# sen-ye/dmvae

Measured on AMD Instinct MI355X. Metric: images/sec DMVAE train step @256x256, higher is better.
Workload: dtype bf16

## Files before the change

dmvae_amd/_lib.py:

```python
from __future__ import annotations

import ctypes
import os
from ctypes import POINTER, Structure, c_char_p, c_double, c_float, c_int, c_int32, c_longlong, c_size_t, c_uint, c_ulonglong, c_void_p

_HERE = os.path.dirname(os.path.abspath(__file__))
LIB_PATH = os.environ.get("DMVAE_LIB") or os.path.join(_HERE, "libdmvae_hip.so")


class ConvDesc(Structure):
    _fields_ = [("n", c_int32), ("h", c_int32), ("w", c_int32), ("cin", c_int32), ("cout", c_int32),
                ("ks", c_int32), ("upsample", c_int32), ("act", c_int32), ("out_f32", c_int32), ("stride", c_int32), ("transposed", c_int32),
                ("w_layout", c_int32)]


class PackEntry(Structure):
    _fields_ = [("src", c_void_p), ("dst", c_void_p), ("dst2", c_void_p),
                ("cout", c_int32), ("cin", c_int32), ("T", c_int32), ("rows_pad", c_int32), ("cols_pad", c_int32), ("mode", c_int32), ("subpixel", c_int32),
                ("reserved", c_int32), ("start", c_ulonglong), ("count", c_ulonglong)]


class WtEntry(Structure):
    _fields_ = [("src", c_void_p), ("dst", c_void_p), ("N", c_int32), ("K", c_int32), ("start", c_uint), ("tiles_x", c_uint)]

# ... 34 lines not shown
    "dmvae_gemm_nt_batched": (c_int, [c_void_p] * 5 + [c_int] * 4 + [c_longlong] * 3 + [c_int, c_int, c_void_p]),
    "dmvae_gemm_tn_batched_workspace": (c_size_t, [c_int, c_int, c_int, c_int]),
    "dmvae_gemm_tn_batched": (c_int, [c_void_p] * 4 + [c_size_t] + [c_int] * 4 + [c_longlong] * 3 + [c_float, c_int, c_void_p]),
    "dmvae_set_dynamic": (c_int, [c_int]),
    "dmvae_linear_rows_supported": (c_int, [c_int, c_int, c_int]),
    "dmvae_linear_rows_bf16": (c_int, [c_void_p] * 4 + [c_int] * 10 + [c_void_p]),
    "dmvae_linear_rows_wgrad": (c_int, [c_void_p] * 4 + [c_int] * 6 + [c_void_p]),
    "dmvae_linear_bf16": (c_int, [c_void_p] * 4 + [c_int] * 10 + [c_void_p]),
    "dmvae_linear_bf16_swiglu_pre": (c_int, [c_void_p] * 5 + [c_int] * 9 + [c_void_p]),
    "dmvae_linear_bf16_sk_supported": (c_int, [c_int] * 5),
    "dmvae_linear_bf16_sk_workspace": (c_size_t, [c_int] * 5),
    "dmvae_linear_bf16_sk": (c_int, [c_void_p] * 5 + [c_size_t] + [c_int] * 11 + [c_void_p]),
    "dmvae_linear_bf16_batched_supported": (c_int, [c_int] * 4),
    "dmvae_linear_bf16_batched": (c_int, [c_void_p] * 3 + [c_int] * 7 + [c_longlong] * 3 + [c_int, c_void_p]),
    "dmvae_linear_bf16_plan": (c_int, [c_int, c_int, c_int, POINTER(c_int), POINTER(c_int)]),
    "dmvae_linear_weight_t_kmajor": (c_int, [c_void_p, c_void_p, c_int, c_int, c_void_p]),
    "dmvae_pack_entry_bytes": (c_size_t, []),
    "dmvae_pack_weights_batched": (c_int, [c_void_p, c_int, c_ulonglong, c_int, c_void_p]),
    "dmvae_softmax_rows_fwd": (c_int, [c_void_p, c_void_p, c_int, c_int, c_float, c_void_p]),
    "dmvae_softmax_rows_bwd": (c_int, [c_void_p, c_void_p, c_void_p, c_int, c_int, c_float, c_void_p]),
    "dmvae_transpose_bf16": (c_int, [c_void_p, c_void_p, c_int, c_int, c_int, c_void_p]),
    "dmvae_pack_conv_weight": (c_int, [c_void_p, c_void_p] + [c_int] * 6 + [c_void_p]),
    "dmvae_pack_conv_weight_v2": (c_int, [c_void_p, c_void_p, c_void_p] + [c_int] * 6 + [c_void_p]),
    "dmvae_conv_halo_applies": (c_int, [POINTER(ConvDesc)]),
    "dmvae_conv_kmajor_applies": (c_int, [POINTER(ConvDesc)]),
    "dmvae_subpixel_weight": (c_int, [c_void_p, c_void_p, c_int, c_int, c_void_p]),
    "dmvae_subpixel_weight_fold": (c_int, [c_void_p, c_void_p, c_int, c_int, c_int, c_void_p]),
    "dmvae_colsum_bf16": (c_int, [c_void_p, c_void_p, c_void_p, c_size_t, c_size_t, c_int, c_int, c_void_p]),
    "dmvae_conv_out_wgrad_workspace": (c_size_t, [c_int, c_int, c_int, c_int, c_int]),
    "dmvae_conv_out_wgrad": (c_int, [c_void_p, c_void_p, c_void_p, c_void_p, c_size_t, c_int, c_int, c_int, c_int, c_int, c_int, c_void_p]),
# ... 209 lines not shown
```

dmvae_amd/csrc/common.h:

```cpp
#pragma once
#include <hip/hip_runtime.h>
#include <stdint.h>

typedef __bf16 bf16;
typedef __attribute__((ext_vector_type(8))) __bf16 bf16x8;
typedef __attribute__((ext_vector_type(4))) __bf16 bf16x4;
typedef __attribute__((ext_vector_type(2))) __bf16 bf16x2;
typedef __attribute__((ext_vector_type(4))) short s16x4;
typedef __attribute__((ext_vector_type(16))) float f32x16;
typedef __attribute__((ext_vector_type(4))) float f32x4;
typedef __attribute__((ext_vector_type(2))) float f32x2;

#define GPTR(p) ((const __attribute__((address_space(1))) void*)(p))
#define LPTR(p) ((__attribute__((address_space(3))) void*)(p))

static __device__ uint4 dmvae_zero_page[4];

void dmvae_set_error(const char* fmt, ...);
#define DMVAE_CHECK_ARG(cond, ...) do { if (!(cond)) { dmvae_set_error(__VA_ARGS__); return -22; } } while (0)
#define DMVAE_CHECK_LAUNCH() do { hipError_t e_ = hipGetLastError(); if (e_ != hipSuccess) { dmvae_set_error("%s:%d launch failed: %s", __FILE__, __LINE__, hipGetErrorString(e_)); return -5; } } while (0)

static inline int grid_for(size_t n, int block, int cap) {
  size_t g = (n + block - 1) / block;
  return (int)(g > (size_t)cap ? cap : (g < 1 ? 1 : g));
// ... 26 lines not shown
}
__device__ __forceinline__ s16x4 tr_read_ordered(const char* p) {
  return __builtin_amdgcn_ds_read_tr16_b64_v4i16((__attribute__((address_space(3))) s16x4*)(p));
}

__device__ __forceinline__ float wave_sum(float v) {
#pragma unroll
  for (int o = 32; o > 0; o >>= 1) v += __shfl_xor(v, o, 64);
  return v;
}
__device__ __forceinline__ float bf2f(bf16 v) { return (float)v; }
__device__ __forceinline__ float sigmoidf_(float x) { return __builtin_amdgcn_rcpf(1.0f + __expf(-x)); }
__device__ __forceinline__ float sigmoid_exact(float x) { return 1.0f / (1.0f + expf(-x)); }

__device__ __forceinline__ float dmvae_gelu_f(float x) {
  const float z = fabsf(x) * 0.70710678118654752f;
  const float t = __builtin_amdgcn_rcpf(__builtin_fmaf(0.3275911f, z, 1.0f));
  float p = __builtin_fmaf(1.061405429f, t, -1.453152027f);
  p = __builtin_fmaf(p, t, 1.421413741f);
  p = __builtin_fmaf(p, t, -0.284496736f);
  p = __builtin_fmaf(p, t, 0.254829592f);
  const float e = p * t * __expf(-z * z);
  return 0.5f * x * (x < 0.f ? e : 2.0f - e);
}

__device__ __forceinline__ unsigned xcd_remap(unsigned flat, unsigned total) {
  const unsigned q = total >> 3, r = total & 7u, x = flat & 7u;
  const unsigned start = x < r ? x * (q + 1) : r * (q + 1) + (x - r) * q;
  return start + (flat >> 3);
}

__device__ __forceinline__ bf16x8 dmvae_ldnt8(const bf16* p) {
  return __builtin_nontemporal_load(reinterpret_cast<const bf16x8*>(p));
}
__device__ __forceinline__ unsigned dmvae_pack_bf16x2(float a, float b) {
  bf16x2 t = {(bf16)a, (bf16)b};
  return *reinterpret_cast<unsigned*>(&t);
}
// ... 28 lines not shown
```

dmvae_amd/csrc/gemm_pp.hip:

```cpp
#include "common.h"
#include "dmvae_hip.h"
#include <cstdlib>
#include <type_traits>

constexpr int GEMM_MAXBUF = 6;

namespace dmvae_gemm_pp {

struct Args {
  const bf16* x;
  const bf16* w;
  const void* bias;
  void* y;
  int M, N, K, lda, ldw, ldy;
  int act, bias_bf16;
  int H;
  unsigned wbytes;
  unsigned wsRow, wsK;
  int ntn, total;
  float inv_ntn;
  int tpb;
  float inv_tpb;
  unsigned sA, sB, sY, xbytes, ybytes;
  unsigned long long* dbg;
  int V, skS, T;
  float* slabs;
  unsigned* counters;
  unsigned slab_bytes;
  void* y2;
  int ldy2;
};

constexpr int SK_COHERENT = 1 | 16;

template <int TM, int TP, int WM, int WP, bool OUT_F32, int NBUF, bool BATCHED = false, bool SK = false>
__global__ __launch_bounds__(WM * WP * 64) void gemm_pp_kernel(Args a) {
#if __HIP_DEVICE_COMPILE__
  constexpr int PF = NBUF - 1;
  static_assert(!(SK && BATCHED) && !(SK && OUT_F32), "SK: single product, bf16 result");
  constexpr int CL = TM / WM / 16, BT = TP / WP / 16;
  constexpr int NW = WM * WP;
  static_assert(NW == 8 && CL * 16 * WM == TM && BT * 16 * WP == TP && CL * BT <= 32 && (CL == 4 || CL == 6 || CL == 8), "wave grid");
  constexpr int TILE_A = TM * 64, TILE_B = TP * 64, SLOT = TILE_A + TILE_B, RING = NBUF * SLOT;
  constexpr int NPA = (TM / 16 + NW - 1) / NW, NPB = (TP / 16 + NW - 1) / NW, NP = NPA + NPB;
  constexpr int CW = CL * 16;
  constexpr int BIAS_OFF = RING, DUMP_OFF = RING + 2048;
// ... 29 lines not shown
    if constexpr (BATCHED) {
      int b = (int)((float)wid * a.inv_tpb);
      int r = wid - b * a.tpb;
      if (r < 0) { b--; r += a.tpb; }
      if (r >= a.tpb) { b++; r -= a.tpb; }
      b0 = __builtin_amdgcn_readfirstlane(b);
      wid = r;
      offA = (unsigned)b0 * a.sA; offB = (unsigned)b0 * a.sB;
    }
    int mt = (int)((float)wid * inv_ntn);
    int nt = wid - mt * a.ntn;
    if (nt < 0) { mt--; nt += a.ntn; }
    if (nt >= a.ntn) { mt++; nt -= a.ntn; }
    m0 = __builtin_amdgcn_readfirstlane(mt) * TP;
    n0 = __builtin_amdgcn_readfirstlane(nt) * TM;
#pragma unroll
    for (int p = 0; p < NPA; p++) {
      const int rl = (wave * NPA + p) * 16 + (lane_c >> 2);
      const int wmr = rl / CW, r = rl % CW, i = r >> 4, c = r & 15;
      int n = n0 + wmr * CW + CL * c + i;
      bool n_ok = n < a.N;
      if (gated) {
        const int hid = (n0 >> 1) + wmr * (CW / 2) + (CL / 2) * c + (i % (CL / 2));
        n = (i < CL / 2 ? 0 : a.H) + hid;
        n_ok = hid < a.H;
      }
      const int ch = (lane_c & 3) ^ swz64(rl);
      vA[p] = (live && rl < TM && n_ok) ? (unsigned)n * a.wsRow + ch * 16u + offA : SENT;
    }
#pragma unroll
// ... 108 lines not shown
    __builtin_amdgcn_sched_barrier(0);
#pragma unroll
    for (int i = 0; i < CL; i++)
#pragma unroll
      for (int j = 0; j < BT; j++)
        asm volatile("v_mfma_f32_16x16x32_bf16 %0, %1, %2, %0" : "+a"(acc[i][j]) : "v"(tf[j]), "v"(wf[i]));
    __builtin_amdgcn_sched_barrier(0);
    __builtin_amdgcn_s_barrier();
    __builtin_amdgcn_sched_barrier(0);
  };
  using W_NO = std::integral_constant<int, -1>; using W_0 = std::integral_constant<int, 0>;
  using W_ST = std::integral_constant<int, (PF - 1) * NP>; using W_TL = std::integral_constant<int, (PF - 1) * NP + 1>;
  using M0_ = std::integral_constant<int, 0>;
  static_assert((PF - 1) * NP + 1 < 64, "vmcnt is a 6-bit counter");

  unsigned work = blockIdx.x;
  if constexpr (SK) { uc = next_unit(); work = (unsigned)uc.tile; }
  {
    unsigned vBiasC;
    calc(work, vAc, vBc, vBiasC, m0c, n0c, b0c);
    issue_bias(vBiasC, 0);
  }
#pragma unroll
  for (int u = 0; u < PF; u++) issue_k(vAc, vBc, (unsigned)(u + (SK ? uc.kb : 0)), u * SLOT);
  wait_vmcnt<0>();

  int tix = 0;
  auto stamp = [&](int k) { if (a.dbg && tid == 0 && tix < 4) a.dbg[((size_t)blockIdx.x * 4 + tix) * 8 + k] = __builtin_amdgcn_s_memtime(); };
  while (work < (unsigned)a.total) {
    stamp(0);
    __builtin_amdgcn_s_barrier();
    {
      const char* bl = smem + BIAS_OFF + par * 1024;
      int lane_b = lane;
      asm volatile("" : "+v"(lane_b));
      const int col = gated ? wm * (CW / 2) + (CL / 2) * (lane_b & 15) : wm * CW + CL * (lane_b & 15);
      const int hop = gated ? TM / 2 - CL / 2 : 0;
      float bv[8] = {0.f, 0.f, 0.f, 0.f, 0.f, 0.f, 0.f, 0.f};
      if (!a.bias || (SK && uc.p != 0)) {
      } else if (a.bias_bf16) {
#pragma unroll
        for (int h = 0; h < CL / 2; h++) {
          const bf16x2 b2 = *reinterpret_cast<const bf16x2*>(bl + (col + (h >= CL / 4 ? hop : 0)) * 2 + h * 4);
// ... 146 lines not shown
                  } else {
                    const unsigned p1 = dmvae_pack_bf16x2(v[0], v[1]), p2 = dmvae_pack_bf16x2(v[2], v[3]);
                    __builtin_amdgcn_raw_buffer_store_b32(p1, rY2, ok2 ? e1 : SENT, 0, 0);
                    __builtin_amdgcn_raw_buffer_store_b32(p2, rY2, ok2 ? e2 : SENT, 0, 0);
                    asm volatile("s_nop 0" :: "v"(p1), "v"(p2));
                  }
                }
              }
#pragma unroll
              for (int i = 0; i < CL / 2; i++) {
                const float x1 = (float)(bf16)v[i], x2 = (float)(bf16)v[CL / 2 + i];
                v[i] = (float)(bf16)(x1 * sigmoidf_(x1)) * x2;
              }
            } else if constexpr (ACT != 0) {
#pragma unroll
              for (int i = 0; i < CL; i++) {
                const float x = (float)(bf16)v[i];
                v[i] = ACT == 5 ? dmvae_gelu_f(x) : x * sigmoidf_(x);
              }
            }
            const int m = row0 + j * 16 + r;
            const bool ok = c_ok && m < a.M;
            const unsigned eo = (unsigned)m * (unsigned)a.ldy + (unsigned)col;
            if constexpr (ACT == 6) {
              if constexpr (CL == 8 && !OUT_F32) {
                const u32x2 o = {dmvae_pack_bf16x2(v[0], v[1]), dmvae_pack_bf16x2(v[2], v[3])};
                __builtin_amdgcn_raw_buffer_store_b64(o, rY, ok ? eo * 2u : SENT, ysoff, 0);
                asm volatile("s_nop 0" :: "v"(o));
              } else if constexpr (CL == 4 && !OUT_F32) {
                const unsigned o = dmvae_pack_bf16x2(v[0], v[1]);
                __builtin_amdgcn_raw_buffer_store_b32(o, rY, ok ? eo * 2u : SENT, ysoff, 0);
                asm volatile("s_nop 0" :: "v"(o));
              }
            } else if constexpr (OUT_F32 && CL == 6) {
// ... 58 lines not shown
#pragma unroll
    for (int p = 0; p < NPA; p++) vAc[p] = vAn[p];
#pragma unroll
    for (int p = 0; p < NPB; p++) vBc[p] = vBn[p];
    m0c = m0n; n0c = n0n; b0c = b0n;
    if constexpr (SK) uc = un;
    par ^= 1;
  }
#endif
}

template <int TM, int TP, int WM, int WP, bool F32, bool BATCHED = false>
int launch(Args a, hipStream_t st, int batch = 1) {
  a.ntn = (a.N + TM - 1) / TM;
  a.tpb = ((a.M + TP - 1) / TP) * a.ntn;
  a.total = a.tpb * batch;
  DMVAE_CHECK_ARG(a.total > 0 && a.total < (1 << 24) && (long long)a.tpb * batch < (1 << 24),
                  "linear_bf16: %lld output tiles (the kernel's tile index arithmetic is exact below 2^24)", (long long)a.tpb * batch);
  a.inv_ntn = 1.0f / (float)a.ntn;
  a.inv_tpb = 1.0f / (float)a.tpb;
  const unsigned grid = a.total > 256 ? 256u : (unsigned)a.total;
  constexpr int slot = (TM + TP) * 64;
  constexpr int fit = (160 * 1024 - 3 * 1024) / slot;
  constexpr int nbuf = fit > GEMM_MAXBUF ? GEMM_MAXBUF : fit;
  static_assert(nbuf >= 4, "LDS");
  constexpr int lds = nbuf * slot + 3 * 1024;
  DMVAE_LDS_OPTIN(lds, gemm_pp_kernel<TM, TP, WM, WP, F32, nbuf, BATCHED>);
  hipLaunchKernelGGL((gemm_pp_kernel<TM, TP, WM, WP, F32, nbuf, BATCHED>), dim3(grid), dim3(WM * WP * 64), lds, st, a);
  DMVAE_CHECK_LAUNCH();
  return 0;
// ... 31 lines not shown
  const int nK = K >> 5;
  if (tiles > SK_MAX_TILES || tiles * nK >= (1ll << 30)) return false;
  if (splits == 0) return tiles * nK / SK_GRID >= 2 * t.minseg && nK >= 2 * t.minseg;
  return nK / splits >= t.minseg && tiles * splits <= 4096;
}

struct Cfg { int tm, tp; float cost; };
static const Cfg g_cfg[] = {
    {256, 256, 1.00f}, {256, 224, 0.94f}, {256, 192, 0.885f}, {256, 160, 0.80f}, {256, 128, 0.67f},
    {128, 448, 1.02f}, {128, 384, 0.93f}, {128, 256, 0.70f},  {192, 256, 0.90f}, {192, 320, 1.12f},
    {192, 128, 0.54f}, {128, 192, 0.54f},
};
constexpr int NCFG = sizeof(g_cfg) / sizeof(g_cfg[0]);

static int g_forced = -1;
static int plan(int M, int N, int K, bool gated = false) {
  const int forced = g_forced;
  if (forced >= 0 && forced < NCFG && !(gated && g_cfg[forced].tm == 192)) return forced;
  (void)K;
  constexpr int NPLAN = 10;
  int best = 0;
  float best_t = 1e30f;
  for (int c = 0; c < NPLAN; c++) {
    if (gated && g_cfg[c].tm == 192) continue;
    const long long tiles = (long long)((M + g_cfg[c].tp - 1) / g_cfg[c].tp) * ((N + g_cfg[c].tm - 1) / g_cfg[c].tm);
    const float frac = (float)tiles / 256.0f, whole = 0.85f * (float)((tiles + 255) / 256);
    const float t = (frac > whole ? frac : whole) * g_cfg[c].cost;
    if (t < best_t * 0.999f) { best_t = t; best = c; }
  }
  return best;
}

template <bool F32>
static int dispatch(int cfg, const Args& a, hipStream_t st) {
  switch (cfg) {
    case 0: return launch<256, 256, 2, 4, F32>(a, st);
    case 1: return launch<256, 224, 4, 2, F32>(a, st);
    case 2: return launch<256, 192, 2, 4, F32>(a, st);
    case 3: return launch<256, 160, 4, 2, F32>(a, st);
    case 4: return launch<256, 128, 4, 2, F32>(a, st);
    case 5: return launch<128, 448, 2, 4, F32>(a, st);
    case 6: return launch<128, 384, 2, 4, F32>(a, st);
    case 7: return launch<128, 256, 2, 4, F32>(a, st);
// ... 3 lines not shown
    default: return launch<128, 192, 2, 4, F32>(a, st);
  }
}

}

static unsigned long long* g_gemm_dbg = nullptr;
extern "C" void dmvae_debug_gemm_timing(void* buf) { g_gemm_dbg = (unsigned long long*)buf; }
extern "C" void dmvae_debug_gemm_cfg(int cfg) { dmvae_gemm_pp::g_forced = cfg; }

extern "C" int dmvae_linear_bf16_plan(int M, int N, int K, int* tile_cols, int* tile_rows) {
  using namespace dmvae_gemm_pp;
  const int c = plan(M, N, K);
  if (tile_cols) *tile_cols = g_cfg[c].tm;
  if (tile_rows) *tile_rows = g_cfg[c].tp;
  return c;
}

extern "C" int dmvae_linear_bf16_batched_supported(int batch, int M, int N, int K) {
  return (batch > 0 && M >= 64 && N > 0 && N % 8 == 0 && K >= 384 && K % 32 == 0) ? 1 : 0;
}
extern "C" int dmvae_linear_bf16_batched(const void* x, const void* w, void* y, int batch, int M, int N, int K, int lda, int ldw, int ldy, long long sx, long long sw,
                                         long long sy, int out_f32, hipStream_t stream) {
  using namespace dmvae_gemm_pp;
  DMVAE_CHECK_ARG(x && w && y, "linear_bf16_batched: null operand");
  DMVAE_CHECK_ARG(dmvae_linear_bf16_batched_supported(batch, M, N, K), "linear_bf16_batched: need K %% 32 == 0, K >= 384, N %% 8 == 0, M >= 64 (batch %d, M %d, N %d, K %d)",
                  batch, M, N, K);
  DMVAE_CHECK_ARG(lda >= K && ldw >= K && ldy >= N && lda % 8 == 0 && ldw % 8 == 0 && ldy % 8 == 0, "linear_bf16_batched: leading dimensions must cover the rows and be multiples of 8");
  DMVAE_CHECK_ARG(sx >= (long long)M * lda && sw >= (long long)N * ldw && sy >= (long long)M * ldy && sx % 8 == 0 && sw % 8 == 0 && sy % 8 == 0,
                  "linear_bf16_batched: batch strides must cover one product's operand and be multiples of 8 elements");
  const long long xb = ((long long)(batch - 1) * sx + (long long)M * lda) * 2, wb = ((long long)(batch - 1) * sw + (long long)N * ldw) * 2;
  const long long yb = ((long long)(batch - 1) * sy + (long long)M * ldy) * (out_f32 ? 4 : 2);
  DMVAE_CHECK_ARG(xb < (1ll << 31) && wb < (1ll << 31) && yb < (1ll << 31), "linear_bf16_batched: operands are addressed through 32-bit buffer offsets (2 GiB each over the whole batch)");
  Args a;
  a.x = (const bf16*)x; a.w = (const bf16*)w; a.bias = nullptr; a.y = y;
  a.M = M; a.N = N; a.K = K; a.lda = lda; a.ldw = ldw; a.ldy = ldy;
  a.act = 0; a.bias_bf16 = 0; a.H = N / 2; a.ntn = 0; a.total = 0; a.inv_ntn = 0.f; a.dbg = nullptr;
  a.V = a.skS = a.T = 0; a.slabs = nullptr; a.counters = nullptr; a.slab_bytes = 0u; a.y2 = nullptr; a.ldy2 = 0;
  a.wbytes = (unsigned)wb; a.xbytes = (unsigned)xb; a.ybytes = (unsigned)yb;
  a.wsRow = (unsigned)ldw * 2u; a.wsK = 64u;
  a.sA = (unsigned)(sw * 2); a.sB = (unsigned)(sx * 2); a.sY = (unsigned)(sy * (out_f32 ? 4 : 2));
  static const int cand[3] = {0, 4, 7};
  int best = 0;
  float best_t = 1e30f;
  for (int i = 0; i < 3; i++) {
    const Cfg& c = g_cfg[cand[i]];
    const long long tiles = (long long)batch * ((M + c.tp - 1) / c.tp) * ((N + c.tm - 1) / c.tm);
    const float frac = (float)tiles / 256.0f, whole = 0.85f * (float)((tiles + 255) / 256);
    const float t = (frac > whole ? frac : whole) * c.cost;
    if (t < best_t * 0.999f) { best_t = t; best = cand[i]; }
  }
  if (out_f32) {
    if (best == 0) return launch<256, 256, 2, 4, true, true>(a, stream, batch);
// ... 25 lines not shown
  DMVAE_CHECK_ARG(act == 0 || act == 1 || act == 5 || act == 6, "linear_bf16_sk: act must be 0 (none), 1 (SiLU), 5 (GELU) or 6 (SwiGLU over the [x1 | x2] halves of N)");
  DMVAE_CHECK_ARG(act != 6 || N % 16 == 0, "linear_bf16_sk: the SwiGLU epilogue needs N %% 16 == 0");
  const long long wb = w_layout == 1 ? (long long)N * K * 2 : (long long)N * ldw * 2;
  DMVAE_CHECK_ARG((long long)M * lda * 2 < (1ll << 31) && wb < (1ll << 31) && (long long)M * ldy * 2 < (1ll << 31),
                  "linear_bf16_sk: operands are addressed through 32-bit buffer offsets (2 GiB each)");
  const size_t need = dmvae_linear_bf16_sk_workspace(M, N, K, splits, tile);
  DMVAE_CHECK_ARG(workspace_bytes >= need && need - SK_COUNTER_BYTES < (1ull << 32), "linear_bf16_sk: workspace too small (need %zu bytes, see dmvae_linear_bf16_sk_workspace)", need);
  Args a;
  a.x = (const bf16*)x; a.w = (const bf16*)w; a.bias = bias; a.y = y;
  a.M = M; a.N = N; a.K = K; a.lda = lda; a.ldw = ldw; a.ldy = ldy;
  a.act = act; a.bias_bf16 = bias_bf16; a.H = N / 2; a.ntn = 0; a.total = 0; a.inv_ntn = 0.f; a.dbg = g_gemm_dbg;
  a.wbytes = (unsigned)wb; a.tpb = 0; a.inv_tpb = 0.f; a.sA = a.sB = a.sY = a.xbytes = a.ybytes = 0u;
  a.wsRow = w_layout == 1 ? 64u : (unsigned)ldw * 2u;
  a.wsK = w_layout == 1 ? (unsigned)N * 64u : 64u;
  a.y2 = nullptr; a.ldy2 = 0;
  a.counters = (unsigned*)workspace;
  a.slabs = (float*)((char*)workspace + SK_COUNTER_BYTES);
  a.slab_bytes = (unsigned)(need - SK_COUNTER_BYTES);
  return launch_sk(a, splits, tile, stream);
}

static int linear_bf16_impl(const void* x, const void* w, const void* bias, void* y, void* y2, int ldy2, int M, int N, int K, int lda, int ldw, int ldy,
                            int act, int bias_bf16, int out_f32, int w_layout, hipStream_t stream);
extern "C" int dmvae_linear_bf16(const void* x, const void* w, const void* bias, void* y, int M, int N, int K, int lda, int ldw, int ldy,
                                 int act, int bias_bf16, int out_f32, int w_layout, hipStream_t stream) {
  return linear_bf16_impl(x, w, bias, y, nullptr, 0, M, N, K, lda, ldw, ldy, act, bias_bf16, out_f32, w_layout, stream);
}
extern "C" int dmvae_linear_bf16_swiglu_pre(const void* x, const void* w, const void* bias, void* g, void* x12, int M, int N, int K, int lda, int ldw, int ldg,
                                            int ldx12, int bias_bf16, int w_layout, hipStream_t stream) {
  DMVAE_CHECK_ARG(x12 && ldx12 >= N && ldx12 % 8 == 0, "linear_bf16_swiglu_pre: x12 must be given with ldx12 >= N, a multiple of 8");
  return linear_bf16_impl(x, w, bias, g, x12, ldx12, M, N, K, lda, ldw, ldg, 6, bias_bf16, 0, w_layout, stream);
}
static int linear_bf16_impl(const void* x, const void* w, const void* bias, void* y, void* y2, int ldy2, int M, int N, int K, int lda, int ldw, int ldy,
                            int act, int bias_bf16, int out_f32, int w_layout, hipStream_t stream) {
  using namespace dmvae_gemm_pp;
  DMVAE_CHECK_ARG(x && w && y, "linear_bf16: null operand");
  DMVAE_CHECK_ARG(M > 0 && N > 0 && K >= 384 && K % 32 == 0 && N % 8 == 0, "linear_bf16: need K %% 32 == 0, K >= 384 and N %% 8 == 0 (M %d, N %d, K %d)", M, N, K);
  DMVAE_CHECK_ARG(w_layout == 0 || w_layout == 1, "linear_bf16: w_layout must be 0 (row-major [N][ldw]) or 1 (K-tile-major [K / 32][N][32])");
  DMVAE_CHECK_ARG(lda >= K && (w_layout == 1 || ldw >= K) && ldy >= (act == 6 ? N / 2 : N) && lda % 8 == 0 && ldw % 8 == 0 && ldy % 8 == 0,
                  "linear_bf16: leading dimensions must cover the rows and be multiples of 8");
  DMVAE_CHECK_ARG(act == 0 || act == 1 || act == 5 || act == 6, "linear_bf16: act must be 0 (none), 1 (SiLU), 5 (GELU) or 6 (SwiGLU over the [x1 | x2] halves of N)");
  DMVAE_CHECK_ARG(act != 6 || (!out_f32 && N % 16 == 0), "linear_bf16: the SwiGLU epilogue writes bf16 and needs N %% 16 == 0");
  const long long wb = w_layout == 1 ? (long long)N * K * 2 : (long long)N * ldw * 2;
  DMVAE_CHECK_ARG((long long)M * lda * 2 < (1ll << 31) && wb < (1ll << 31) && (long long)M * ldy * (out_f32 ? 4 : 2) < (1ll << 31),
                  "linear_bf16: operands are addressed through 32-bit buffer offsets (2 GiB each)");
  Args a;
  a.x = (const bf16*)x; a.w = (const bf16*)w; a.bias = bias; a.y = y;
  a.M = M; a.N = N; a.K = K; a.lda = lda; a.ldw = ldw; a.ldy = ldy;
  a.act = act; a.bias_bf16 = bias_bf16; a.H = N / 2; a.ntn = 0; a.total = 0; a.inv_ntn = 0.f; a.dbg = g_gemm_dbg;
  a.V = a.skS = a.T = 0; a.slabs = nullptr; a.counters = nullptr; a.slab_bytes = 0u; a.y2 = y2; a.ldy2 = ldy2;
  DMVAE_CHECK_ARG(!y2 || (long long)M * ldy2 * 2 < (1ll << 31), "linear_bf16_swiglu_pre: x12 is addressed through 32-bit buffer offsets (2 GiB)");
  a.wbytes = (unsigned)wb; a.tpb = 0; a.inv_tpb = 0.f; a.sA = a.sB = a.sY = a.xbytes = a.ybytes = 0u;
  a.wsRow = w_layout == 1 ? 64u : (unsigned)ldw * 2u;
  a.wsK = w_layout == 1 ? (unsigned)N * 64u : 64u;
  const int cfg = plan(M, N, K, act == 6);
  return out_f32 ? dispatch<true>(cfg, a, stream) : dispatch<false>(cfg, a, stream);
}
```

dmvae_amd/functional.py:

```python
from __future__ import annotations

from typing import Optional
import os

import weakref

import torch

from . import ops, parity
from .ops import bf16, f32

_EPOCH = [0]


def bump_weight_epoch() -> None:
    _EPOCH[0] += 1


def _epoch_of(w) -> int:
    return getattr(w, "_dmvae_epoch", _EPOCH)[0]


def packed(w: torch.Tensor, for_dgrad: bool = False, rows_pad: int = 0, cols_pad: int = 0, frozen: bool = False,
           transposed: bool = False, subpixel: bool = False, kmajor: bool = False) -> torch.Tensor:
# ... 776 lines not shown
SPLITK = 3
SPLITK_MIN_K = 3072
_SPLITK_ACTIVE = [0]


def _use_splitk(m: int, n: int, k: int) -> int:
    s_ = _SPLITK_ACTIVE[0]
    if s_ < 2 or parity.on() or not (2048 <= m <= 6144) or k < SPLITK_MIN_K:
        return 0
    tiles = ((m + 255) // 256) * ((n + 255) // 256)
    if tiles > 100:
        return 0
    return s_ if ops.linear_sk_supported(m, n, k, s_) else 0


def linear(x: torch.Tensor, w: torch.Tensor, b: Optional[torch.Tensor] = None, act: int = ops.ACT_NONE) -> torch.Tensor:
    bb = None if b is None else (b if b.dtype == bf16 else _bf(b))
    k = x.shape[-1]
    n = w.shape[0]
    m = x.numel() // k
    x = _c(x)
    if x.dtype != bf16:
        x = x.to(bf16)
    if m <= 64 and act in (ops.ACT_NONE, ops.ACT_SILU) and ops.linear_rows_supported(m, n, k) and not parity.on():
        return ops.linear_rows(x.view(m, k), (w if w.dtype == bf16 else _bf(w)).view(n, k), bb, act).view(*x.shape[:-1], n)
    sk = _use_splitk(m, n, k) if act == ops.ACT_NONE else 0
    if sk:
        return ops.linear_sk(x.view(m, k), (w if w.dtype == bf16 else _bf(w)).view(n, k), bb, splits=sk).view(*x.shape[:-1], n)
    if ops.linear_supported(m, n, k) and (act != ops.ACT_SWIGLU or n % 16 == 0):
        if isinstance(w, torch.nn.Parameter) and not w.requires_grad and not hasattr(w, "_dmvae_epoch") and w.dim() == 2:
            return ops.linear_bf16(x, _bf_km(w), bb, act)
        return ops.linear_bf16(x, (w if w.dtype == bf16 else _bf(w)).view(n, k), bb, act)
    wb = w if w.dtype == bf16 else _bf(w)
    x2, w2 = x.view(m, k), wb.view(n, k)
    if k % 32 != 0 or n % 4 != 0:
        kp, np_ = (-k) % 32, (-n) % 4
        x2 = torch.nn.functional.pad(x2, (0, kp))
        w2 = torch.nn.functional.pad(w2, (0, kp, 0, np_))
        bb = None if bb is None else torch.nn.functional.pad(bb, (0, np_))
    y = ops.gemm_nt(x2, w2, None if bb is None else bb.float())[:, :n]
    if act == ops.ACT_GELU:
        y = ops.gelu(y)
    elif act == ops.ACT_SILU:
        y = ops.silu(y)
    elif act == ops.ACT_SWIGLU:
        y = ops.swiglu(_c(y))
    return y.reshape(*x.shape[:-1], y.shape[-1])
# ... 718 lines not shown
```

dmvae_amd/models/vit_fast.py:

```python
import torch
import torch.nn.functional as F

from .. import ops


def patch_embed_gemm(vit, x: torch.Tensor) -> torch.Tensor:
    w = vit.patch_embed.proj.weight
    b_, c, hh, ww = x.shape
    p = w.shape[-1]
    assert hh % p == 0 and ww % p == 0, "image size must be a multiple of the patch size"
    patches = x.view(b_, c, hh // p, p, ww // p, p).permute(0, 2, 4, 1, 3, 5).reshape(b_, (hh // p) * (ww // p), c * p * p)
    if not torch.is_grad_enabled():
        from ..functional import linear
        return linear(patches.to(torch.bfloat16), _w(w).view(w.shape[0], -1), _w(vit.patch_embed.proj.bias))
    from ..functional import LinearFn
    return LinearFn.apply(patches, w.view(w.shape[0], -1), vit.patch_embed.proj.bias)


def _w(p: torch.Tensor) -> torch.Tensor:
    if p.dtype == torch.bfloat16:
        return p
    from ..functional import _bf
    return _bf(p)


@torch.no_grad()
def frozen_forward_features(vit, x: torch.Tensor, key_depths=None, pos_embed=None):
    from ..functional import linear
    t = patch_embed_gemm(vit, x).float()
    t = torch.cat([vit.cls_token.expand(t.shape[0], -1, -1).float(), t], dim=1) + (vit.pos_embed if pos_embed is None else pos_embed).float()
    taps, last_tap = [], (max(key_depths) if key_depths is not None else -1)
    t = t.contiguous()
    b, s, c = t.shape
    hn = ops.layernorm_bf16(t, vit.blocks[0].norm1.weight, vit.blocks[0].norm1.bias, vit.blocks[0].norm1.eps)
    nblk = len(vit.blocks)
    for i, blk in enumerate(vit.blocks):
        nh = blk.attn.num_heads
        hd = c // nh
        qkv = linear(hn, blk.attn.qkv.weight, blk.attn.qkv.bias)
        if hd == 64:
            o = ops.attention_qkv(qkv, nh, hd ** -0.5)
        else:
            from .._stock import require_opt_in
            require_opt_in("vit_fast.forward_features (attention)", f"head dim {hd}: the fused attention kernels take head dim 64")
            qkv = qkv.reshape(b, s, 3, nh, hd).permute(2, 0, 3, 1, 4)
            att = ops.softmax_rows_bf16(qkv[0] @ qkv[1].transpose(-2, -1), hd ** -0.5)
            o = (att @ qkv[2]).transpose(1, 2).reshape(b, s, c)
        o = linear(o, blk.attn.proj.weight, blk.attn.proj.bias)
        hn = ops.scale_residual_layernorm_(t, o.contiguous(), blk.ls1.gamma, blk.norm2.weight, blk.norm2.bias, blk.norm2.eps)
        h = linear(hn, blk.mlp.fc1.weight, blk.mlp.fc1.bias, act=ops.ACT_GELU)
        o = linear(h, blk.mlp.fc2.weight, blk.mlp.fc2.bias)
        if i == last_tap:
            taps.append(ops.scale_residual_(t, o.contiguous(), blk.ls2.gamma))
            return taps
        nxt = vit.blocks[i + 1].norm1 if i + 1 < nblk else vit.norm
        hn = ops.scale_residual_layernorm_(t, o, blk.ls2.gamma, nxt.weight, nxt.bias, nxt.eps)
        if key_depths is not None and i in key_depths:
            taps.append(t.clone())
    if key_depths is not None:
        raise ValueError(f"key_depths {tuple(key_depths)}: the model has {nblk} blocks")
    return hn


def hip_path_supported(vit, seq_len: int) -> bool:
    c = vit.embed_dim
    nh = vit.blocks[0].attn.num_heads
    return c in (256, 384, 512, 768, 1024, 1280, 1536) and c // nh == 64


NOGRAD_FUSED = True


def frozen_taps_with_input_grad(vit, x: torch.Tensor, key_depths, pos_embed=None):
    from ..functional import VitBlockDxFn
    t = patch_embed_gemm(vit, x)
    t = torch.cat([vit.cls_token.expand(t.shape[0], -1, -1).float(), t.float()], dim=1) + (vit.pos_embed if pos_embed is None else pos_embed).float()
    t = t.contiguous()
    taps = []
    for i, blk in enumerate(vit.blocks[:max(key_depths) + 1]):
        t = VitBlockDxFn.apply(t, blk.norm1.weight, blk.norm1.bias, blk.attn.qkv.weight, blk.attn.qkv.bias, blk.attn.proj.weight, blk.attn.proj.bias,
                               blk.ls1.gamma, blk.norm2.weight, blk.norm2.bias, blk.mlp.fc1.weight, blk.mlp.fc1.bias, blk.mlp.fc2.weight,
                               blk.mlp.fc2.bias, blk.ls2.gamma, blk.attn.num_heads, blk.norm1.eps)
        if i in key_depths:
            taps.append(t)
# ... 61 lines not shown
```

dmvae_amd/ops.py:

```python
from __future__ import annotations

import ctypes
import os
from typing import Optional, Sequence, Tuple

import torch

from . import _lib, parity
from ._lib import ConvDesc, check

bf16 = torch.bfloat16
f32 = torch.float32

ACT_NONE, ACT_SILU, ACT_RELU, ACT_RELU_GATE, ACT_LEAKY, ACT_GELU = 0, 1, 2, 3, 4, 5
ACT_SWIGLU = 6


def _stream() -> int:
    return torch.cuda.current_stream().cuda_stream


def _req(t: torch.Tensor, dtype, name: str) -> torch.Tensor:
    if not t.is_cuda:
        raise _lib.DmvaeHipError(f"{name}: expected a GPU tensor; dmvae_amd has no CPU path")
# ... 295 lines not shown
    m = x.numel() // k
    bias_bf16 = 0
    if bias is not None:
        if bias.dtype == bf16:
            bias_bf16 = 1
        _req(bias, bf16 if bias_bf16 else f32, "bias")
        assert bias.numel() == n
    ny = n // 2 if act == ACT_SWIGLU else n
    y = torch.empty(*x.shape[:-1], ny, dtype=f32 if out_f32 else bf16, device=x.device)
    timing = KERNEL_TIMING
    if timing is not None:
        e0 = torch.cuda.Event(enable_timing=True)
        e0.record()
    check(_lib.lib().dmvae_linear_bf16(x.data_ptr(), w.data_ptr(), _ptr(bias), y.data_ptr(), m, n, k, k, k, ny, act, bias_bf16, int(out_f32), int(kmajor),
                                       _stream()), "linear_bf16")
    if timing is not None:
        e1 = torch.cuda.Event(enable_timing=True)
        e1.record()
        timing.append(("gemm_pp_kernel", e0, e1, 2.0 * m * n * k))
    return y


def linear_swiglu_pre(x: torch.Tensor, w: torch.Tensor, bias: Optional[torch.Tensor] = None):
    x = _req(x, bf16, "x")
    w = _req(w, bf16, "w")
    k = x.shape[-1]
    kmajor = w.dim() == 3
    n = w.shape[1] if kmajor else w.shape[0]
    assert (w.shape[0] * 32 == k and w.shape[2] == 32) if kmajor else (w.shape[1] == k), (x.shape, w.shape)
    m = x.numel() // k
# ... 2005 lines not shown
```

include/dmvae_hip.h:

```cpp
#ifndef DMVAE_HIP_H
#define DMVAE_HIP_H

#include <stddef.h>
#include <stdint.h>

#ifdef __cplusplus
extern "C" {
#endif

typedef struct ihipStream_t* dmvae_stream_t;

const char* dmvae_last_error(void);
int dmvae_abi_version(void);


typedef struct dmvae_conv_desc {
  int32_t n, h, w;
  int32_t cin, cout;
  int32_t ks;
  int32_t upsample;
  int32_t act;
  int32_t out_f32;
  int32_t stride;
  int32_t transposed;
// ... 74 lines not shown
size_t dmvae_gemm_tn_batched_workspace(int M, int N, int K, int batch);
int dmvae_gemm_tn_batched(const void* A, const void* B, void* C, void* workspace, size_t workspace_bytes, int M,
                          int N, int K, int batch, long long a_bs, long long b_bs, long long c_bs, float alpha,
                          int out_f32, dmvae_stream_t stream);

int dmvae_linear_rows_supported(int M, int N, int K);
int dmvae_linear_rows_bf16(const void* x, const void* w, const void* bias, void* y, int M, int N, int K, int ldx, int ldw, int ldy, int act,
                           int bias_bf16, int out_f32, int w_layout, dmvae_stream_t stream);
int dmvae_linear_rows_wgrad(const void* dy, const void* x, void* dw, void* db, int M, int N, int K, int lddy, int ldx, int accumulate, dmvae_stream_t stream);

int dmvae_set_dynamic(int on);

int dmvae_linear_bf16(const void* x, const void* w, const void* bias, void* y, int M, int N, int K, int lda, int ldw, int ldy,
                      int act, int bias_bf16, int out_f32, int w_layout, dmvae_stream_t stream);
int dmvae_linear_bf16_plan(int M, int N, int K, int* tile_cols, int* tile_rows);
int dmvae_linear_bf16_batched_supported(int batch, int M, int N, int K);
int dmvae_linear_bf16_batched(const void* x, const void* w, void* y, int batch, int M, int N, int K, int lda, int ldw, int ldy, long long sx, long long sw,
                              long long sy, int out_f32, dmvae_stream_t stream);
int dmvae_linear_bf16_swiglu_pre(const void* x, const void* w, const void* bias, void* g, void* x12, int M, int N, int K, int lda, int ldw, int ldg,
                                 int ldx12, int bias_bf16, int w_layout, dmvae_stream_t stream);

int dmvae_linear_bf16_sk_supported(int M, int N, int K, int splits, int tile);
size_t dmvae_linear_bf16_sk_workspace(int M, int N, int K, int splits, int tile);
int dmvae_linear_bf16_sk(const void* x, const void* w, const void* bias, void* y, void* workspace, size_t workspace_bytes, int splits, int tile,
                         int M, int N, int K, int lda, int ldw, int ldy, int act, int bias_bf16, int w_layout, dmvae_stream_t stream);
int dmvae_linear_weight_t_kmajor(const void* w, void* out, int N, int K, dmvae_stream_t stream);

int dmvae_softmax_rows_fwd(const void* s, void* p, int rows, int cols, float scale, dmvae_stream_t stream);
int dmvae_softmax_rows_bwd(const void* dp, const void* p, void* ds, int rows, int cols, float scale,
                           dmvae_stream_t stream);
// ... 365 lines not shown
```

Before: 502.2.

## Add segmented GEMM mode so ViT fc1 tiles skip CLS rows via strip pass

Adds a segmented linear mode for the frozen ViT feature extractor's fc1 GEMM. Each sequence of s rows has its leading CLS row handled by a small MFMA strip pass run before the main tiled loop. The main tiles then cover only the remaining 256-multiple token rows, so per-image sequences of 257 tokens no longer spill into a partially filled tile. The planner weighs the strip cost against tile savings, and the GELU epilogue is also rewritten with contraction off and an explicit fma.

```diff
diff --git a/dmvae_amd/_lib.py b/dmvae_amd/_lib.py
--- a/dmvae_amd/_lib.py
+++ b/dmvae_amd/_lib.py
@@ -72,6 +72,8 @@
     "dmvae_linear_bf16_batched_supported": (c_int, [c_int] * 4),
     "dmvae_linear_bf16_batched": (c_int, [c_void_p] * 3 + [c_int] * 7 + [c_longlong] * 3 + [c_int, c_void_p]),
     "dmvae_linear_bf16_plan": (c_int, [c_int, c_int, c_int, POINTER(c_int), POINTER(c_int)]),
+    "dmvae_linear_bf16_seg": (c_int, [c_void_p] * 4 + [c_int] * 13 + [c_void_p]),
+    "dmvae_linear_bf16_seg_plan": (c_int, [c_int] * 6 + [POINTER(c_int)] * 3),
     "dmvae_linear_weight_t_kmajor": (c_int, [c_void_p, c_void_p, c_int, c_int, c_void_p]),
     "dmvae_pack_entry_bytes": (c_size_t, []),
     "dmvae_pack_weights_batched": (c_int, [c_void_p, c_int, c_ulonglong, c_int, c_void_p]),
diff --git a/dmvae_amd/csrc/common.h b/dmvae_amd/csrc/common.h
--- a/dmvae_amd/csrc/common.h
+++ b/dmvae_amd/csrc/common.h
@@ -64,14 +64,15 @@
 __device__ __forceinline__ float sigmoid_exact(float x) { return 1.0f / (1.0f + expf(-x)); }
 
 __device__ __forceinline__ float dmvae_gelu_f(float x) {
+#pragma clang fp contract(off)
   const float z = fabsf(x) * 0.70710678118654752f;
   const float t = __builtin_amdgcn_rcpf(__builtin_fmaf(0.3275911f, z, 1.0f));
   float p = __builtin_fmaf(1.061405429f, t, -1.453152027f);
   p = __builtin_fmaf(p, t, 1.421413741f);
   p = __builtin_fmaf(p, t, -0.284496736f);
   p = __builtin_fmaf(p, t, 0.254829592f);
-  const float e = p * t * __expf(-z * z);
-  return 0.5f * x * (x < 0.f ? e : 2.0f - e);
+  const float pt = p * t, ex = __expf(-z * z);
+  return 0.5f * x * (x < 0.f ? pt * ex : __builtin_fmaf(-ex, pt, 2.0f));
 }
 
 __device__ __forceinline__ unsigned xcd_remap(unsigned flat, unsigned total) {
diff --git a/dmvae_amd/csrc/gemm_pp.hip b/dmvae_amd/csrc/gemm_pp.hip
--- a/dmvae_amd/csrc/gemm_pp.hip
+++ b/dmvae_amd/csrc/gemm_pp.hip
@@ -29,7 +29,18 @@
   unsigned slab_bytes;
   void* y2;
   int ldy2;
+  int seg_rows, seg_skip, nseg, seg_tps;
+  float inv_tps;
 };
+
+template <int ACT>
+__device__ __forceinline__ float act_value(float v) {
+  if constexpr (ACT == 0) return v;
+  else {
+    const float x = (float)(bf16)v;
+    return ACT == 5 ? dmvae_gelu_f(x) : x * sigmoidf_(x);
+  }
+}
 
 constexpr int SK_COHERENT = 1 | 16;
 
@@ -89,6 +100,16 @@
     if (nt >= a.ntn) { mt++; nt -= a.ntn; }
     m0 = __builtin_amdgcn_readfirstlane(mt) * TP;
     n0 = __builtin_amdgcn_readfirstlane(nt) * TM;
+    if constexpr (!BATCHED && !SK) {
+      if (a.seg_rows) {
+        const int mtu = __builtin_amdgcn_readfirstlane(mt);
+        int sg = (int)((float)mtu * a.inv_tps);
+        int r = mtu - sg * a.seg_tps;
+        if (r < 0) { sg--; r += a.seg_tps; }
+        if (r >= a.seg_tps) { sg++; r -= a.seg_tps; }
+        m0 = __builtin_amdgcn_readfirstlane(sg * a.seg_rows + a.seg_skip + r * TP);
+      }
+    }
 #pragma unroll
     for (int p = 0; p < NPA; p++) {
       const int rl = (wave * NPA + p) * 16 + (lane_c >> 2);
@@ -227,6 +248,8 @@
   using M0_ = std::integral_constant<int, 0>;
   static_assert((PF - 1) * NP + 1 < 64, "vmcnt is a 6-bit counter");
 
+  int tix = 0;
+  auto stamp = [&](int k) { if (a.dbg && tid == 0 && tix < 4) a.dbg[((size_t)blockIdx.x * 4 + tix) * 8 + k] = __builtin_amdgcn_s_memtime(); };
   unsigned work = blockIdx.x;
   if constexpr (SK) { uc = next_unit(); work = (unsigned)uc.tile; }
   {
@@ -236,10 +259,80 @@
   }
 #pragma unroll
   for (int u = 0; u < PF; u++) issue_k(vAc, vBc, (unsigned)(u + (SK ? uc.kb : 0)), u * SLOT);
+
+  if constexpr (!BATCHED && !SK) {
+    if (a.seg_rows) {
+      stamp(4);
+      constexpr int SD = 12;
+      const int R = a.nseg * a.seg_skip, RB = (R + 15) >> 4, CB = (a.N + 15) >> 4;
+      const int ncl = (CB - (int)blockIdx.x + (int)gridDim.x - 1) / (int)gridDim.x;
+      const int c16 = lane & 15, g4 = lane >> 4;
+      auto strip_row = [&](int s_) -> int { const int sg = s_ / a.seg_skip; return sg * a.seg_rows + (s_ - sg * a.seg_skip); };
+      for (int lu = wave; lu < ncl * RB; lu += NW) {
+        const int ci = lu / RB, rb = lu - ci * RB;
+        const int n = ((int)blockIdx.x + ci * (int)gridDim.x) * 16 + c16;
+        const int s_in = rb * 16 + c16;
+        const unsigned vX = s_in < R ? (unsigned)strip_row(s_in) * (unsigned)a.lda * 2u + (unsigned)g4 * 16u : SENT;
+        const unsigned vW = n < a.N ? (unsigned)n * a.wsRow + (unsigned)g4 * 16u : SENT;
+        float bv = 0.f;
+        if (a.bias) {
+          if (a.bias_bf16) {
+            const unsigned short raw = (unsigned short)__builtin_amdgcn_raw_buffer_load_b16(rBias, n < a.N ? (unsigned)n * 2u : SENT, 0, 0);
+            bv = (float)*reinterpret_cast<const bf16*>(&raw);
+          } else {
+            bv = __builtin_bit_cast(float, __builtin_amdgcn_raw_buffer_load_b32(rBias, n < a.N ? (unsigned)n * 4u : SENT, 0, 0));
+          }
+        }
+        f32x4 sacc = {bv, bv, bv, bv};
+        int k0 = 0;
+        auto steps = [&](auto NBc) __attribute__((always_inline)) {
+          constexpr int NB = decltype(NBc)::value;
+          u32x4 xa[NB], wb[NB];
+#pragma unroll
+          for (int u = 0; u < NB; u++) {
+            xa[u] = __builtin_amdgcn_raw_buffer_load_b128(rB, vX, (unsigned)(k0 + u) * 64u, 0);
+            wb[u] = __builtin_amdgcn_raw_buffer_load_b128(rA, vW, (unsigned)(k0 + u) * a.wsK, 0);
+          }
+          __builtin_amdgcn_sched_barrier(0);
+#pragma unroll
+          for (int u = 0; u < NB; u++)
+            sacc = __builtin_amdgcn_mfma_f32_16x16x32_bf16(*reinterpret_cast<const bf16x8*>(&xa[u]), *reinterpret_cast<const bf16x8*>(&wb[u]), sacc, 0, 0, 0);
+          k0 += NB;
+        };
+#pragma unroll 1
+        while (k0 + SD <= nK) steps(std::integral_constant<int, SD>{});
+        if (k0 + 8 <= nK) steps(std::integral_constant<int, 8>{});
+        if (k0 + 4 <= nK) steps(std::integral_constant<int, 4>{});
+        if (k0 + 2 <= nK) steps(std::integral_constant<int, 2>{});
+        if (k0 < nK) steps(std::integral_constant<int, 1>{});
+        auto put = [&](auto ACTc) __attribute__((always_inline)) {
+          constexpr int ACT = decltype(ACTc)::value;
+#pragma unroll
+          for (int r = 0; r < 4; r++) {
+            const int s_out = rb * 16 + 4 * g4 + r;
+            const bool ok = s_out < R && n < a.N;
+            const unsigned eo = (unsigned)strip_row(s_out) * (unsigned)a.ldy + (unsigned)n;
+            const float v = act_value<ACT>(sacc[r]);
+            if constexpr (OUT_F32) {
+              const unsigned o = __builtin_bit_cast(unsigned, v);
+              __builtin_amdgcn_raw_buffer_store_b32(o, rY, ok ? eo * 4u : SENT, 0, 0);
+              asm volatile("s_nop 0" :: "v"(o));
+            } else {
+              const unsigned short o = (unsigned short)(dmvae_pack_bf16x2(v, 0.f) & 0xffffu);
+              __builtin_amdgcn_raw_buffer_store_b16(o, rY, ok ? eo * 2u : SENT, 0, 0);
+              asm volatile("s_nop 0" :: "v"(o));
+            }
+          }
+        };
+        if (a.act == 0) put(std::integral_constant<int, 0>{});
+        else if (a.act == 5) put(std::integral_constant<int, 5>{});
+        else put(std::integral_constant<int, 1>{});
+      }
+      stamp(5);
+    }
+  }
   wait_vmcnt<0>();
 
-  int tix = 0;
-  auto stamp = [&](int k) { if (a.dbg && tid == 0 && tix < 4) a.dbg[((size_t)blockIdx.x * 4 + tix) * 8 + k] = __builtin_amdgcn_s_memtime(); };
   while (work < (unsigned)a.total) {
     stamp(0);
     __builtin_amdgcn_s_barrier();
@@ -416,10 +509,7 @@
               }
             } else if constexpr (ACT != 0) {
 #pragma unroll
-              for (int i = 0; i < CL; i++) {
-                const float x = (float)(bf16)v[i];
-                v[i] = ACT == 5 ? dmvae_gelu_f(x) : x * sigmoidf_(x);
-              }
+              for (int i = 0; i < CL; i++) v[i] = act_value<ACT>(v[i]);
             }
             const int m = row0 + j * 16 + r;
             const bool ok = c_ok && m < a.M;
@@ -508,6 +598,11 @@
 int launch(Args a, hipStream_t st, int batch = 1) {
   a.ntn = (a.N + TM - 1) / TM;
   a.tpb = ((a.M + TP - 1) / TP) * a.ntn;
+  if (a.seg_rows) {
+    a.seg_tps = (a.seg_rows - a.seg_skip) / TP;
+    a.inv_tps = 1.0f / (float)a.seg_tps;
+    a.tpb = a.nseg * a.seg_tps * a.ntn;
+  }
   a.total = a.tpb * batch;
   DMVAE_CHECK_ARG(a.total > 0 && a.total < (1 << 24) && (long long)a.tpb * batch < (1 << 24),
                   "linear_bf16: %lld output tiles (the kernel's tile index arithmetic is exact below 2^24)", (long long)a.tpb * batch);
@@ -569,9 +664,19 @@
 constexpr int NCFG = sizeof(g_cfg) / sizeof(g_cfg[0]);
 
 static int g_forced = -1;
-static int plan(int M, int N, int K, bool gated = false) {
+struct Seg { int rows, skip, n; };
+constexpr float STRIP_COST = 0.22f;
+static bool seg_fits(const Seg* seg, int M, int tp) {
+  return seg && seg->rows > 0 && seg->skip > 0 && seg->skip < seg->rows && seg->n > 0 && (long long)seg->n * seg->rows == M && (seg->rows - seg->skip) % tp == 0;
+}
+static int plan(int M, int N, int K, bool gated = false, const Seg* seg = nullptr, bool* use_seg = nullptr) {
+  if (use_seg) *use_seg = false;
+  if (gated) seg = nullptr;
   const int forced = g_forced;
-  if (forced >= 0 && forced < NCFG && !(gated && g_cfg[forced].tm == 192)) return forced;
+  if (forced >= 0 && forced < NCFG && !(gated && g_cfg[forced].tm == 192)) {
+    if (use_seg) *use_seg = seg_fits(seg, M, g_cfg[forced].tp);
+    return forced;
+  }
   (void)K;
   constexpr int NPLAN = 10;
   int best = 0;
@@ -581,7 +686,15 @@
     const long long tiles = (long long)((M + g_cfg[c].tp - 1) / g_cfg[c].tp) * ((N + g_cfg[c].tm - 1) / g_cfg[c].tm);
     const float frac = (float)tiles / 256.0f, whole = 0.85f * (float)((tiles + 255) / 256);
     const float t = (frac > whole ? frac : whole) * g_cfg[c].cost;
-    if (t < best_t * 0.999f) { best_t = t; best = c; }
+    if (t < best_t * 0.999f) { best_t = t; best = c; if (use_seg) *use_seg = false; }
+    if (seg_fits(seg, M, g_cfg[c].tp)) {
+      const long long stiles = (long long)seg->n * ((seg->rows - seg->skip) / g_cfg[c].tp) * ((N + g_cfg[c].tm - 1) / g_cfg[c].tm);
+      const long long grid = stiles > 256 ? 256 : stiles;
+      const long long blocks = (((N + 15) / 16 + grid - 1) / grid) * (((long long)seg->n * seg->skip + 15) / 16);
+      const float sfrac = (float)stiles / 256.0f, swhole = 0.85f * (float)((stiles + 255) / 256);
+      const float ts = (sfrac > swhole ? sfrac : swhole) * g_cfg[c].cost + STRIP_COST * (float)((blocks + 7) / 8);
+      if (ts < best_t * 0.999f) { best_t = ts; best = c; if (use_seg) *use_seg = true; }
+    }
   }
   return best;
 }
@@ -615,6 +728,16 @@
   const int c = plan(M, N, K);
   if (tile_cols) *tile_cols = g_cfg[c].tm;
   if (tile_rows) *tile_rows = g_cfg[c].tp;
+  return c;
+}
+extern "C" int dmvae_linear_bf16_seg_plan(int M, int N, int K, int seg_rows, int seg_skip, int nseg, int* tile_cols, int* tile_rows, int* segmented) {
+  using namespace dmvae_gemm_pp;
+  const Seg seg = {seg_rows, seg_skip, nseg};
+  bool us = false;
+  const int c = plan(M, N, K, false, &seg, &us);
+  if (tile_cols) *tile_cols = g_cfg[c].tm;
+  if (tile_rows) *tile_rows = g_cfg[c].tp;
+  if (segmented) *segmented = us ? 1 : 0;
   return c;
 }
 
@@ -638,6 +761,7 @@
   a.M = M; a.N = N; a.K = K; a.lda = lda; a.ldw = ldw; a.ldy = ldy;
   a.act = 0; a.bias_bf16 = 0; a.H = N / 2; a.ntn = 0; a.total = 0; a.inv_ntn = 0.f; a.dbg = nullptr;
   a.V = a.skS = a.T = 0; a.slabs = nullptr; a.counters = nullptr; a.slab_bytes = 0u; a.y2 = nullptr; a.ldy2 = 0;
+  a.seg_rows = a.seg_skip = a.nseg = a.seg_tps = 0; a.inv_tps = 0.f;
   a.wbytes = (unsigned)wb; a.xbytes = (unsigned)xb; a.ybytes = (unsigned)yb;
   a.wsRow = (unsigned)ldw * 2u; a.wsK = 64u;
   a.sA = (unsigned)(sw * 2); a.sB = (unsigned)(sx * 2); a.sY = (unsigned)(sy * (out_f32 ? 4 : 2));
@@ -693,6 +817,7 @@
   a.wsRow = w_layout == 1 ? 64u : (unsigned)ldw * 2u;
   a.wsK = w_layout == 1 ? (unsigned)N * 64u : 64u;
   a.y2 = nullptr; a.ldy2 = 0;
+  a.seg_rows = a.seg_skip = a.nseg = a.seg_tps = 0; a.inv_tps = 0.f;
   a.counters = (unsigned*)workspace;
   a.slabs = (float*)((char*)workspace + SK_COUNTER_BYTES);
   a.slab_bytes = (unsigned)(need - SK_COUNTER_BYTES);
@@ -700,10 +825,22 @@
 }
 
 static int linear_bf16_impl(const void* x, const void* w, const void* bias, void* y, void* y2, int ldy2, int M, int N, int K, int lda, int ldw, int ldy,
-                            int act, int bias_bf16, int out_f32, int w_layout, hipStream_t stream);
+                            int act, int bias_bf16, int out_f32, int w_layout, hipStream_t stream, const dmvae_gemm_pp::Seg* seg = nullptr);
 extern "C" int dmvae_linear_bf16(const void* x, const void* w, const void* bias, void* y, int M, int N, int K, int lda, int ldw, int ldy,
                                  int act, int bias_bf16, int out_f32, int w_layout, hipStream_t stream) {
   return linear_bf16_impl(x, w, bias, y, nullptr, 0, M, N, K, lda, ldw, ldy, act, bias_bf16, out_f32, w_layout, stream);
+}
+extern "C" int dmvae_linear_bf16_seg(const void* x, const void* w, const void* bias, void* y, int M, int N, int K, int lda, int ldw, int ldy,
+                                     int act, int bias_bf16, int out_f32, int w_layout, int seg_rows, int seg_skip, int nseg, hipStream_t stream) {
+  using namespace dmvae_gemm_pp;
+  DMVAE_CHECK_ARG(seg_rows > 0 && nseg > 0 && seg_skip > 0 && seg_skip < seg_rows && (long long)nseg * seg_rows == (long long)M,
+                  "linear_bf16_seg: need M == nseg * seg_rows and 0 < seg_skip < seg_rows (M %d, seg_rows %d, seg_skip %d, nseg %d)", M, seg_rows, seg_skip, nseg);
+  DMVAE_CHECK_ARG(act != 6, "linear_bf16_seg: the SwiGLU epilogue is not available over segments");
+  const Seg seg = {seg_rows, seg_skip, nseg};
+  bool any = false;
+  for (int c = 0; c < NCFG; c++) any = any || seg_fits(&seg, M, g_cfg[c].tp);
+  DMVAE_CHECK_ARG(any, "linear_bf16_seg: seg_rows - seg_skip = %d is a multiple of no tile's rows (128, 160, 192, 224, 256, 320, 384, 448)", seg_rows - seg_skip);
+  return linear_bf16_impl(x, w, bias, y, nullptr, 0, M, N, K, lda, ldw, ldy, act, bias_bf16, out_f32, w_layout, stream, &seg);
 }
 extern "C" int dmvae_linear_bf16_swiglu_pre(const void* x, const void* w, const void* bias, void* g, void* x12, int M, int N, int K, int lda, int ldw, int ldg,
                                             int ldx12, int bias_bf16, int w_layout, hipStream_t stream) {
@@ -711,7 +848,7 @@
   return linear_bf16_impl(x, w, bias, g, x12, ldx12, M, N, K, lda, ldw, ldg, 6, bias_bf16, 0, w_layout, stream);
 }
 static int linear_bf16_impl(const void* x, const void* w, const void* bias, void* y, void* y2, int ldy2, int M, int N, int K, int lda, int ldw, int ldy,
-                            int act, int bias_bf16, int out_f32, int w_layout, hipStream_t stream) {
+                            int act, int bias_bf16, int out_f32, int w_layout, hipStream_t stream, const dmvae_gemm_pp::Seg* seg) {
   using namespace dmvae_gemm_pp;
   DMVAE_CHECK_ARG(x && w && y, "linear_bf16: null operand");
   DMVAE_CHECK_ARG(M > 0 && N > 0 && K >= 384 && K % 32 == 0 && N % 8 == 0, "linear_bf16: need K %% 32 == 0, K >= 384 and N %% 8 == 0 (M %d, N %d, K %d)", M, N, K);
@@ -732,6 +869,9 @@
   a.wbytes = (unsigned)wb; a.tpb = 0; a.inv_tpb = 0.f; a.sA = a.sB = a.sY = a.xbytes = a.ybytes = 0u;
   a.wsRow = w_layout == 1 ? 64u : (unsigned)ldw * 2u;
   a.wsK = w_layout == 1 ? (unsigned)N * 64u : 64u;
-  const int cfg = plan(M, N, K, act == 6);
+  bool use_seg = false;
+  const int cfg = plan(M, N, K, act == 6, seg, &use_seg);
+  a.seg_rows = a.seg_skip = a.nseg = a.seg_tps = 0; a.inv_tps = 0.f;
+  if (use_seg) { a.seg_rows = seg->rows; a.seg_skip = seg->skip; a.nseg = seg->n; }
   return out_f32 ? dispatch<true>(cfg, a, stream) : dispatch<false>(cfg, a, stream);
 }
diff --git a/dmvae_amd/functional.py b/dmvae_amd/functional.py
--- a/dmvae_amd/functional.py
+++ b/dmvae_amd/functional.py
@@ -814,7 +814,7 @@
     return s_ if ops.linear_sk_supported(m, n, k, s_) else 0
 
 
-def linear(x: torch.Tensor, w: torch.Tensor, b: Optional[torch.Tensor] = None, act: int = ops.ACT_NONE) -> torch.Tensor:
+def linear(x: torch.Tensor, w: torch.Tensor, b: Optional[torch.Tensor] = None, act: int = ops.ACT_NONE, segments=None) -> torch.Tensor:
     bb = None if b is None else (b if b.dtype == bf16 else _bf(b))
     k = x.shape[-1]
     n = w.shape[0]
@@ -829,8 +829,12 @@
         return ops.linear_sk(x.view(m, k), (w if w.dtype == bf16 else _bf(w)).view(n, k), bb, splits=sk).view(*x.shape[:-1], n)
     if ops.linear_supported(m, n, k) and (act != ops.ACT_SWIGLU or n % 16 == 0):
         if isinstance(w, torch.nn.Parameter) and not w.requires_grad and not hasattr(w, "_dmvae_epoch") and w.dim() == 2:
-            return ops.linear_bf16(x, _bf_km(w), bb, act)
-        return ops.linear_bf16(x, (w if w.dtype == bf16 else _bf(w)).view(n, k), bb, act)
+            wop = _bf_km(w)
+        else:
+            wop = (w if w.dtype == bf16 else _bf(w)).view(n, k)
+        if segments is not None and act != ops.ACT_SWIGLU:
+            return ops.linear_bf16_seg(x, wop, bb, segments, act)
+        return ops.linear_bf16(x, wop, bb, act)
     wb = w if w.dtype == bf16 else _bf(w)
     x2, w2 = x.view(m, k), wb.view(n, k)
     if k % 32 != 0 or n % 4 != 0:
diff --git a/dmvae_amd/models/vit_fast.py b/dmvae_amd/models/vit_fast.py
--- a/dmvae_amd/models/vit_fast.py
+++ b/dmvae_amd/models/vit_fast.py
@@ -26,6 +26,7 @@
 
 @torch.no_grad()
 def frozen_forward_features(vit, x: torch.Tensor, key_depths=None, pos_embed=None):
+    from .. import parity
     from ..functional import linear
     t = patch_embed_gemm(vit, x).float()
     t = torch.cat([vit.cls_token.expand(t.shape[0], -1, -1).float(), t], dim=1) + (vit.pos_embed if pos_embed is None else pos_embed).float()
@@ -48,7 +49,8 @@
             o = (att @ qkv[2]).transpose(1, 2).reshape(b, s, c)
         o = linear(o, blk.attn.proj.weight, blk.attn.proj.bias)
         hn = ops.scale_residual_layernorm_(t, o.contiguous(), blk.ls1.gamma, blk.norm2.weight, blk.norm2.bias, blk.norm2.eps)
-        h = linear(hn, blk.mlp.fc1.weight, blk.mlp.fc1.bias, act=ops.ACT_GELU)
+        seg = (s, 1, b) if SEGMENTED_FC1 and (s - 1) % 256 == 0 and s > 1 and not parity.on() else None
+        h = linear(hn, blk.mlp.fc1.weight, blk.mlp.fc1.bias, act=ops.ACT_GELU, segments=seg)
         o = linear(h, blk.mlp.fc2.weight, blk.mlp.fc2.bias)
         if i == last_tap:
             taps.append(ops.scale_residual_(t, o.contiguous(), blk.ls2.gamma))
@@ -68,6 +70,7 @@
     return c in (256, 384, 512, 768, 1024, 1280, 1536) and c // nh == 64
 
 
+SEGMENTED_FC1 = True
 NOGRAD_FUSED = True
 
 
diff --git a/dmvae_amd/ops.py b/dmvae_amd/ops.py
--- a/dmvae_amd/ops.py
+++ b/dmvae_amd/ops.py
@@ -333,6 +333,52 @@
         e0.record()
     check(_lib.lib().dmvae_linear_bf16(x.data_ptr(), w.data_ptr(), _ptr(bias), y.data_ptr(), m, n, k, k, k, ny, act, bias_bf16, int(out_f32), int(kmajor),
                                        _stream()), "linear_bf16")
+    if timing is not None:
+        e1 = torch.cuda.Event(enable_timing=True)
+        e1.record()
+        timing.append(("gemm_pp_kernel", e0, e1, 2.0 * m * n * k))
+    return y
+
+
+def linear_seg_plan(m: int, n: int, k: int, seg_rows: int, seg_skip: int, nseg: int) -> Tuple[int, int, int, bool]:
+    tc, tr, sg = ctypes.c_int(0), ctypes.c_int(0), ctypes.c_int(0)
+    idx = _lib.lib().dmvae_linear_bf16_seg_plan(m, n, k, seg_rows, seg_skip, nseg, ctypes.byref(tc), ctypes.byref(tr), ctypes.byref(sg))
+    return idx, tc.value, tr.value, bool(sg.value)
+
+
+def linear_bf16_seg(x: torch.Tensor, w: torch.Tensor, bias: Optional[torch.Tensor], segments: Tuple[int, int, int], act: int = ACT_NONE,
+                    out_f32: bool = False, out: Optional[torch.Tensor] = None) -> torch.Tensor:
+    x = _req(x, bf16, "x")
+    w = _req(w, bf16, "w")
+    k = x.shape[-1]
+    kmajor = w.dim() == 3
+    if kmajor:
+        assert w.shape[2] == 32 and w.shape[0] * 32 == k, (x.shape, w.shape)
+        n = w.shape[1]
+    else:
+        assert w.dim() == 2 and w.shape[1] == k, (x.shape, w.shape)
+        n = w.shape[0]
+    m = x.numel() // k
+    assert act != ACT_SWIGLU, "linear_bf16_seg: no SwiGLU epilogue over segments"
+    bias_bf16 = 0
+    if bias is not None:
+        bias_bf16 = int(bias.dtype == bf16)
+        _req(bias, bf16 if bias_bf16 else f32, "bias")
+        assert bias.numel() == n
+    if out is None:
+        y = torch.empty(*x.shape[:-1], n, dtype=f32 if out_f32 else bf16, device=x.device)
+        ldy = n
+    else:
+        y = out
+        assert y.dim() == 2 and tuple(y.shape) == (m, n) and y.stride(1) == 1 and y.dtype == (f32 if out_f32 else bf16) and y.device == x.device, (y.shape, y.stride())
+        ldy = y.stride(0)
+    seg_rows, seg_skip, nseg = (int(v) for v in segments)
+    timing = KERNEL_TIMING
+    if timing is not None:
+        e0 = torch.cuda.Event(enable_timing=True)
+        e0.record()
+    check(_lib.lib().dmvae_linear_bf16_seg(x.data_ptr(), w.data_ptr(), _ptr(bias), y.data_ptr(), m, n, k, k, k, ldy, act, bias_bf16, int(out_f32), int(kmajor),
+                                           seg_rows, seg_skip, nseg, _stream()), "linear_bf16_seg")
     if timing is not None:
         e1 = torch.cuda.Event(enable_timing=True)
         e1.record()
diff --git a/include/dmvae_hip.h b/include/dmvae_hip.h
--- a/include/dmvae_hip.h
+++ b/include/dmvae_hip.h
@@ -112,6 +112,9 @@
 int dmvae_linear_bf16(const void* x, const void* w, const void* bias, void* y, int M, int N, int K, int lda, int ldw, int ldy,
                       int act, int bias_bf16, int out_f32, int w_layout, dmvae_stream_t stream);
 int dmvae_linear_bf16_plan(int M, int N, int K, int* tile_cols, int* tile_rows);
+int dmvae_linear_bf16_seg(const void* x, const void* w, const void* bias, void* y, int M, int N, int K, int lda, int ldw, int ldy,
+                          int act, int bias_bf16, int out_f32, int w_layout, int seg_rows, int seg_skip, int nseg, dmvae_stream_t stream);
+int dmvae_linear_bf16_seg_plan(int M, int N, int K, int seg_rows, int seg_skip, int nseg, int* tile_cols, int* tile_rows, int* segmented);
 int dmvae_linear_bf16_batched_supported(int batch, int M, int N, int K);
 int dmvae_linear_bf16_batched(const void* x, const void* w, void* y, int batch, int M, int N, int K, int lda, int ldw, int ldy, long long sx, long long sw,
                               long long sy, int out_f32, dmvae_stream_t stream);
```

Result: no change. 504.2 (median of 6 runs) (+0.4%).
